# laboshinl/loam_velodyne

Measured on AMD Instinct MI355X. Metric: sweeps/sec (64-ring, 1M-pt map): feature extraction + odometry + scan-to-map registration, higher is better.
Workload: dtype f32

## Files before the change

loam_velodyne_amd/csrc/registration.hip:

```cpp
#include "registration.hpp"
#include "pinned_copy.hpp"
#include <atomic>
#include <chrono>
#include "scan.hpp"
#include "voxel.hpp"

namespace loamx {

__global__ __launch_bounds__(256) void k_stack(const float4* __restrict__ in, const float4* const* __restrict__ src, uint32_t n,
                                               const uint32_t* __restrict__ seg_off, uint32_t nseg, const Pose* __restrict__ poses,
                                               float inv_corner, float inv_surf, float4* __restrict__ stack, int* __restrict__ ijk,
                                               int* __restrict__ seg_minmax) {
  const uint32_t i = blockIdx.x * blockDim.x + threadIdx.x;
  const bool active = i < n;
  uint32_t seg = 0;
  int ix = 0, iy = 0, iz = 0;
  if (active) {
    seg = vox_find_seg(seg_off, nseg, i);
    const Pose T = poses[seg >> 1];
    const float4 p = src ? src[seg][i - seg_off[seg]] : in[i];
    float x = p.x, y = p.y, z = p.z;
    to_map(T, x, y, z);
    to_be_mapped(T, x, y, z);
    stack[i] = make_float4(x, y, z, p.w);
// ... 757 lines not shown

static double host_us() {
  return std::chrono::duration<double, std::micro>(std::chrono::steady_clock::now().time_since_epoch()).count();
}
struct Registrar::RunTrace {
  bool on;
  double t0, front = 0, first_gn = 0, callback = 0;
  int looks = 0;
};
#ifdef LOAMX_PROF_GN
static DevBuf<unsigned long long> g_gn_dbg;
#endif

void Registrar::enqueue_full(int mode) {
  if (!n_full_) return;
  if (mode == 1 && ++full_tag_ == 0u) full_tag_ = 1u;
  const uint32_t* skip = run_.vb_unchecked ? vb_.d_fail_word() : nullptr;
  hipLaunchKernelGGL(k_transform_full, dim3((n_full_ + 255) / 256), dim3(256), 0, st_, full_.p, n_full_, d_full_off_, n_sweeps_, poses_.p,
                     stats_.p, full_done_.p, mode, full_tag_, skip, vb_.epoch());
}

void Registrar::enqueue_front(bool legacy) {
  const uint32_t ns = n_sweeps_, nseg = 2 * ns, n = n_in_;
  hipLaunchKernelGGL(k_pose_init, dim3((ns + 63) / 64), dim3(64), 0, st_, d_guess_, ns, poses_.p, stats_.p, vox_.seg_minmax(), arrive_.p,
                     full_done_.p);
  if (n == 0) {
    LX_HIP(hipMemsetAsync(ds_off_.p, 0, sizeof(uint32_t) * (nseg + 1), st_));
    return;
  }
  if (legacy) {
    const uint32_t nb = (n + 255) / 256;
    hipLaunchKernelGGL(k_stack, dim3(nb), dim3(256), 0, st_, in_.p, d_src_, n, d_seg_off_, nseg, poses_.p, 1.0f / params.corner_leaf,
                       1.0f / params.surf_leaf, stack_.p, vox_.ijk(), vox_.seg_minmax());
    vox_.sort_reduce(stack_.p, nullptr, n, d_seg_off_, nseg, ds_pts_.p, ds_off_.p);
  } else {
    vb_.run(in_.p, d_src_, n, d_seg_off_, h_seg_off_.data(), nseg, poses_.p, 1.0f / params.corner_leaf, 1.0f / params.surf_leaf, stack_.p,
            ds_pts_.p, ds_off_.p);
  }
}

bool Registrar::wait_for_mirrors() {
  const bool no_poll = diag_env("LOAMX_NO_MIRROR_POLL") != nullptr;
  if (no_poll) { LX_HIP(hipEventSynchronize(ev_look_)); return false; }
  const uint32_t ns = n_sweeps_;
  const volatile SweepStats* hs = h_stats_.p;
  for (unsigned spin = 0;; spin++) {
    bool all = true;
    for (uint32_t k = 0; k < ns && all; k++) all = hs[k].done != 0;
    if (all) {
      std::atomic_thread_fence(std::memory_order_acquire);
      for (uint32_t k = 0; k < ns && all; k++) {
        SweepStats st;
        Pose T;
        memcpy(&st, (const void*)&h_stats_.p[k], sizeof(st));
        memcpy(&T, (const void*)&h_poses_.p[k], sizeof(T));
        all = st.pad1 == mirror_check_word(st, T);
      }
      if (all) return true;
    }
    if ((spin & 15) == 15) {
// ... 385 lines not shown
```

loam_velodyne_amd/csrc/voxbucket.hip:

```cpp
#include "voxbucket.hpp"
#include "scan.hpp"
#include "voxel.hpp"

namespace loamx {

struct VbArgs {
  const float4* in;
  const float4* const* src;
  const uint32_t* seg_off;
  const Pose* poses;
  VbSeg* segs;
  unsigned long long* lo;
  uint32_t* bseg;
  int* box;
  uint32_t* cnt;
  uint32_t* heads;
  uint32_t* ctl;
  uint32_t* h_fail;
  uint32_t* elems;
  float4* stack;
  float4* out;
  uint32_t* out_off;
  uint32_t n, nseg, nb, epoch;
  float inv_even, inv_odd;
  unsigned long long* dbg;
};

__device__ inline uint32_t vb_bits(unsigned long long v) { return v ? 64u - (uint32_t)__builtin_clzll(v) : 0u; }
__device__ inline void vb_fail(const VbArgs& A, int reason) {
  A.ctl[0] = A.epoch;
  A.h_fail[0] = A.epoch;
  A.h_fail[2 + reason] = A.epoch;
}
__device__ inline void vb_fail_reduce(const VbArgs& A, int reason) {
  vb_fail(A, reason);
  __hip_atomic_store(&A.ctl[0], A.epoch, __ATOMIC_RELAXED, __HIP_MEMORY_SCOPE_AGENT);
}
__device__ inline uint32_t vb_arrive(const VbArgs& A) {
  xchg_stores_done();
  return __hip_atomic_fetch_add(&A.ctl[1], 1u, __ATOMIC_RELAXED, __HIP_MEMORY_SCOPE_AGENT);
}
__device__ inline void vb_arrive_last(const VbArgs& A, uint32_t before) {
  if (before + 1u != A.nb) return;
  __hip_atomic_store(&A.ctl[1], 0u, __ATOMIC_RELAXED, __HIP_MEMORY_SCOPE_AGENT);
  if (__hip_atomic_load(&A.ctl[0], __ATOMIC_RELAXED, __HIP_MEMORY_SCOPE_AGENT) != A.epoch) return;
  for (uint32_t s = 0; s <= A.nseg; s++) __hip_atomic_store(&A.out_off[s], 0u, __ATOMIC_RELAXED, __HIP_MEMORY_SCOPE_AGENT);
}
constexpr int VB_OFF = 1 << 20;
__device__ inline bool vb_voxel(float v, float inv, int& i) {
  const float f = floorf(v * inv);
  if (!(fabsf(f) < (float)VB_OFF)) return false;
  i = (int)f;
  return true;
}
__device__ inline unsigned long long vb_key(int ix, int iy, int iz) {
  return ((unsigned long long)(uint32_t)(iz + VB_OFF) << 42) | ((unsigned long long)(uint32_t)(iy + VB_OFF) << 21) | (unsigned long long)(uint32_t)(ix + VB_OFF);
}

__global__ __launch_bounds__(VB_SAMPLE) void k_vb_plan(const VbArgs A) {
  __shared__ unsigned long long s_key[VB_SAMPLE], s_sorted[VB_SAMPLE];
  __shared__ uint32_t s_scan[17];
  __shared__ uint32_t s_bad;
  const int tid = (int)threadIdx.x;
  const uint32_t seg = blockIdx.x;
  const uint32_t a0 = A.seg_off[seg], ns = A.seg_off[seg + 1] - a0;
  const float4* __restrict__ pts = A.src ? A.src[seg] : A.in + a0;
  const float inv = (seg & 1) ? A.inv_odd : A.inv_even;
  uint32_t bucket0;
  {
    uint32_t part = 0;
    for (uint32_t s = (uint32_t)tid; s < seg; s += VB_SAMPLE) {
      const uint32_t m = A.seg_off[s + 1] - A.seg_off[s];
      part += m ? (m + VB_T - 1) / VB_T : 1u;
    }
    uint32_t tot;
    (void)block_excl_scan(part, s_scan, tot);
    bucket0 = tot;
  }
  const uint32_t nbuckets = ns ? (ns + VB_T - 1) / VB_T : 1u;
  const uint32_t m = ns < (uint32_t)VB_SAMPLE ? ns : (uint32_t)VB_SAMPLE;
  if (tid == 0) s_bad = nbuckets > (uint32_t)VB_SAMPLE ? 2u : 0u;
  __syncthreads();
  unsigned long long key = ~0ull;
  if (nbuckets > 1u && (uint32_t)tid < m) {
    const float4 p = pts[(uint32_t)(((unsigned long long)tid * ns) / m)];
    int v[3];
    if (vb_voxel(p.x, inv, v[0]) && vb_voxel(p.y, inv, v[1]) && vb_voxel(p.z, inv, v[2])) key = vb_key(v[0], v[1], v[2]);
    else atomicOr(&s_bad, 1u);
  }
  s_key[tid] = key;
  __syncthreads();
  if (nbuckets > 1u && (uint32_t)tid < m) {
    uint32_t r = 0;
    for (uint32_t u = 0; u < m; u++) {
      const unsigned long long k = s_key[u];
      r += (k < key || (k == key && u < (uint32_t)tid)) ? 1u : 0u;
    }
    s_sorted[r] = key;
  }
  __syncthreads();
  const uint32_t bad = s_bad;
  if (bad && tid == 0) vb_fail(A, (bad & 2u) ? 1 : 0);
  for (uint32_t k = (uint32_t)tid; k < nbuckets && k < (uint32_t)VB_SAMPLE; k += VB_SAMPLE) {
    A.lo[bucket0 + k] = (k == 0u || bad) ? 0ull : s_sorted[(uint32_t)(((unsigned long long)k * m) / nbuckets)];
    A.bseg[bucket0 + k] = seg;
    A.cnt[bucket0 + k] = 0u;
    A.heads[bucket0 + k] = 0u;
  }
  if (tid < 6) A.box[6 * seg + tid] = tid < 3 ? 2147483647 : (-2147483647 - 1);
  if (tid == 0) {
    VbSeg P;
    P.bucket0 = bucket0;
    P.nbuckets = bad ? 0u : nbuckets;
    P.pos_bits = vb_bits(ns ? (unsigned long long)(ns - 1) : 0ull);
    if (P.pos_bits == 0) P.pos_bits = 1;
    P.pad = 0u;
    A.segs[seg] = P;
  }
}

__global__ __launch_bounds__(256) void k_vb_stack(const VbArgs A) {
  __shared__ unsigned long long s_lo[64];
  __shared__ uint32_t s_tag[256], s_cnt[256], s_gbase[256];
  const uint32_t i = blockIdx.x * blockDim.x + threadIdx.x;
  const int lane = (int)(threadIdx.x & 63);
  const uint32_t lead = vox_find_seg(A.seg_off, A.nseg, blockIdx.x * blockDim.x);
  const VbSeg PL = A.segs[lead];
  if (threadIdx.x < 64) s_lo[threadIdx.x] = threadIdx.x < PL.nbuckets ? A.lo[PL.bucket0 + threadIdx.x] : ~0ull;
  s_tag[threadIdx.x] = 0xffffffffu;
  s_cnt[threadIdx.x] = 0u;
  __syncthreads();
  bool act = i < A.n;
  uint32_t g = 0u, pos = 0u;
  if (act) {
    const uint32_t seg = vox_find_seg(A.seg_off, A.nseg, i);
    const uint32_t a0 = A.seg_off[seg];
    const Pose T = A.poses[seg >> 1];
    const float4 p = A.src ? A.src[seg][i - a0] : A.in[i];
    float x = p.x, y = p.y, z = p.z;
    to_map(T, x, y, z);
    to_be_mapped(T, x, y, z);
    A.stack[i] = make_float4(x, y, z, p.w);
    const float inv = (seg & 1) ? A.inv_odd : A.inv_even;
    int v[3];
    const VbSeg P = seg == lead ? PL : A.segs[seg];
    if (!(vb_voxel(x, inv, v[0]) && vb_voxel(y, inv, v[1]) && vb_voxel(z, inv, v[2])) || P.nbuckets == 0u) {
      vb_fail(A, 0);
      act = false;
    } else {
      const unsigned long long key = vb_key(v[0], v[1], v[2]);
      uint32_t lo = 0u, hi = P.nbuckets;
      if (seg == lead && P.nbuckets <= 64u) {
        while (hi - lo > 1u) { const uint32_t mid = (lo + hi) >> 1; if (s_lo[mid] <= key) lo = mid; else hi = mid; }
      } else {
        const unsigned long long* __restrict__ sp = A.lo + P.bucket0;
        while (hi - lo > 1u) { const uint32_t mid = (lo + hi) >> 1; if (sp[mid] <= key) lo = mid; else hi = mid; }
      }
      g = P.bucket0 + lo;
      pos = i - a0;
    }
  }
  unsigned long long rem = __ballot(act);
  uint32_t slot = 0u;
  bool direct = false;
  while (rem) {
    const int l0 = __builtin_ctzll(rem);
    const uint32_t g0 = (uint32_t)__shfl((int)g, l0, 64);
    const unsigned long long m = __ballot(act && g == g0);
    uint32_t base = 0u, dir = 0u;
    if (lane == l0) {
      const uint32_t h = g0 & 255u;
      const uint32_t old = atomicCAS(&s_tag[h], 0xffffffffu, g0);
      if (old == 0xffffffffu || old == g0) base = atomicAdd(&s_cnt[h], (uint32_t)__popcll(m));
      else { base = atomicAdd(&A.cnt[g0], (uint32_t)__popcll(m)); dir = 1u; }
    }
    base = (uint32_t)__shfl((int)base, l0, 64);
    dir = (uint32_t)__shfl((int)dir, l0, 64);
    if (act && g == g0) { slot = base + (uint32_t)__popcll(m & ((1ull << lane) - 1ull)); direct = dir != 0u; }
    rem &= ~m;
  }
  __syncthreads();
  if (s_tag[threadIdx.x] != 0xffffffffu) s_gbase[threadIdx.x] = atomicAdd(&A.cnt[s_tag[threadIdx.x]], s_cnt[threadIdx.x]);
  __syncthreads();
  if (act) {
    if (!direct) slot += s_gbase[g & 255u];
    if (slot < (uint32_t)VB_CAP) A.elems[(size_t)g * VB_CAP + slot] = pos;
    else vb_fail(A, 5);
  }
}

constexpr uint32_t VB_SPIN_LIMIT = 1u << 20;
#ifdef LOAMX_PROF_VB
#define VB_TS(k) do { if (threadIdx.x == 0) A.dbg[(size_t)blockIdx.x * 16 + (k)] = wall_clock64(); } while (0)
#else
#define VB_TS(k) do { } while (0)
#endif
constexpr int VB_THREADS = VB_CAP / 8, VB_WAVES = VB_THREADS / 64;

__global__ __launch_bounds__(VB_THREADS) void k_vb_reduce(const VbArgs A) {
  __shared__ float4 s_buf[VB_CAP + 1];
  unsigned long long* s_w = (unsigned long long*)s_buf;
  __shared__ uint32_t s_hbits[VB_CAP / 32 + 1];
  __shared__ uint32_t s_wcnt[VB_WAVES][256];
  __shared__ uint32_t s_base[256];
  __shared__ uint32_t s_scan[17];
  __shared__ int s_box[6];
  const int tid = (int)threadIdx.x, lane = tid & 63, wid = tid >> 6;
  const uint32_t b = blockIdx.x;
  VB_TS(0);
  if (__hip_atomic_load(&A.ctl[0], __ATOMIC_RELAXED, __HIP_MEMORY_SCOPE_AGENT) == A.epoch) {
    if (tid == 0) {
      __hip_atomic_store(&A.heads[b], 1u, __ATOMIC_RELAXED, __HIP_MEMORY_SCOPE_AGENT);
      vb_arrive_last(A, vb_arrive(A));
    }
    return;
  }
  const uint32_t seg = A.bseg[b];
  const uint32_t c = min(A.cnt[b], (uint32_t)VB_CAP);
  const VbSeg P = A.segs[seg];
  const uint32_t sbeg = A.seg_off[seg];
  const float inv = (seg & 1) ? A.inv_odd : A.inv_even;
  const uint32_t* __restrict__ e = A.elems + (size_t)b * VB_CAP;
  const uint32_t pbits = P.pos_bits;
  const unsigned long long pmask = (1ull << pbits) - 1ull;
  if (tid < 6) s_box[tid] = tid < 3 ? 2147483647 : (-2147483647 - 1);
  __syncthreads();
  uint32_t pos8[8];
  int vx[8], vy[8], vz[8];
  {
    float4 pt[8];
#pragma unroll
    for (int j = 0; j < 8; j++) {
      const uint32_t i = (uint32_t)(wid * 512 + j * 64 + lane);
      pos8[j] = i < c ? e[i] : 0u;
    }
#pragma unroll
    for (int j = 0; j < 8; j++) {
      const uint32_t i = (uint32_t)(wid * 512 + j * 64 + lane);
      pt[j] = i < c ? A.stack[sbeg + pos8[j]] : make_float4(0.f, 0.f, 0.f, 0.f);
    }
    int mn[3] = {2147483647, 2147483647, 2147483647}, mx[3] = {-2147483647 - 1, -2147483647 - 1, -2147483647 - 1};
#pragma unroll
    for (int j = 0; j < 8; j++) {
      const uint32_t i = (uint32_t)(wid * 512 + j * 64 + lane);
      vx[j] = vy[j] = vz[j] = 0;
      if (i < c) {
        (void)vb_voxel(pt[j].x, inv, vx[j]); (void)vb_voxel(pt[j].y, inv, vy[j]); (void)vb_voxel(pt[j].z, inv, vz[j]);
        mn[0] = vx[j] < mn[0] ? vx[j] : mn[0]; mx[0] = vx[j] > mx[0] ? vx[j] : mx[0];
        mn[1] = vy[j] < mn[1] ? vy[j] : mn[1]; mx[1] = vy[j] > mx[1] ? vy[j] : mx[1];
        mn[2] = vz[j] < mn[2] ? vz[j] : mn[2]; mx[2] = vz[j] > mx[2] ? vz[j] : mx[2];
      }
    }
#pragma unroll
    for (int a = 0; a < 3; a++) {
#pragma unroll
      for (int d = 32; d > 0; d >>= 1) {
        const int lo = __shfl_xor(mn[a], d, 64), hi = __shfl_xor(mx[a], d, 64);
        mn[a] = lo < mn[a] ? lo : mn[a];
        mx[a] = hi > mx[a] ? hi : mx[a];
      }
    }
    if (lane == 0 && (uint32_t)(wid * 512) < c) {
#pragma unroll
      for (int a = 0; a < 3; a++) { atomicMin(&s_box[a], mn[a]); atomicMax(&s_box[3 + a], mx[a]); }
    }
  }
  __syncthreads();
  VB_TS(1);
  unsigned long long dimx = 1ull, dimy = 1ull, dimz = 1ull;
  int bx0 = 0, by0 = 0, bz0 = 0;
  if (c) {
    bx0 = s_box[0]; by0 = s_box[1]; bz0 = s_box[2];
    dimx = (unsigned long long)(s_box[3] - bx0 + 1); dimy = (unsigned long long)(s_box[4] - by0 + 1); dimz = (unsigned long long)(s_box[5] - bz0 + 1);
    if (tid < 6) {
      if (tid < 3) atomicMin(&A.box[6 * seg + tid], s_box[tid]); else atomicMax(&A.box[6 * seg + tid], s_box[tid]);
    }
  }
  const uint32_t key_bits = vb_bits(dimx * dimy * dimz - 1ull);
  const uint32_t total_bits = (key_bits ? key_bits : 1u) + pbits;
  if (total_bits > 63u) {
    if (tid == 0) vb_fail_reduce(A, 3);
  }
  const uint32_t npass = total_bits > 63u ? 0u : (total_bits + 7u) / 8u;
  unsigned long long w[8];
#pragma unroll
  for (int j = 0; j < 8; j++) {
    const uint32_t i = (uint32_t)(wid * 512 + j * 64 + lane);
    const unsigned long long lin = (unsigned long long)(vx[j] - bx0) + dimx * ((unsigned long long)(vy[j] - by0) + dimy * (unsigned long long)(vz[j] - bz0));
    w[j] = i < c ? ((lin << pbits) | (unsigned long long)pos8[j]) : ~0ull;
  }
  const bool wave_has = (uint32_t)(wid * 512) < c;
  if (npass == 0u) {
#pragma unroll
    for (int j = 0; j < 8; j++) {
      const uint32_t i = (uint32_t)(wid * 512 + j * 64 + lane);
      if (i < c) s_w[i] = w[j];
    }
    __syncthreads();
  }
  for (uint32_t p = 0; p < npass; p++) {
    const uint32_t shift = 8u * p;
    VB_TS(2 + (p < 7u ? p : 7u));
    if (tid < 256) {
#pragma unroll
      for (int k = 0; k < VB_WAVES; k++) s_wcnt[k][tid] = 0u;
    }
    __syncthreads();
    uint32_t rank[8];
#pragma unroll
    for (int j = 0; j < 8; j++) rank[j] = 0u;
    if (wave_has) {
#pragma unroll
      for (int j = 0; j < 8; j++) {
        const uint32_t i = (uint32_t)(wid * 512 + j * 64 + lane);
        const bool in = i < c;
        const uint32_t d = (uint32_t)((w[j] >> shift) & 255ull);
        unsigned long long m = __ballot(in);
#pragma unroll
        for (int bit = 0; bit < 8; bit++) {
          const unsigned long long bal = __ballot((d >> bit) & 1u);
          m &= ((d >> bit) & 1u) ? bal : ~bal;
        }
        const unsigned long long below = m & ((1ull << lane) - 1ull);
        const int leader = __builtin_ctzll(m | (1ull << 63));
        uint32_t old = 0u;
        if (in && lane == leader) {
          old = s_wcnt[wid][d];
          s_wcnt[wid][d] = old + (uint32_t)__popcll(m);
        }
        old = (uint32_t)__shfl((int)old, leader, 64);
        rank[j] = old + (uint32_t)__popcll(below);
        __builtin_amdgcn_wave_barrier();
      }
    }
    __syncthreads();
    {
      uint32_t run = 0u;
      if (tid < 256) {
#pragma unroll
        for (int k = 0; k < VB_WAVES; k++) { const uint32_t v = s_wcnt[k][tid]; s_wcnt[k][tid] = run; run += v; }
      }
      uint32_t tot;
      const uint32_t ex = block_excl_scan(run, s_scan, tot);
      if (tid < 256) s_base[tid] = ex;
    }
    __syncthreads();
    if (wave_has) {
#pragma unroll
      for (int j = 0; j < 8; j++) {
        const uint32_t i = (uint32_t)(wid * 512 + j * 64 + lane);
        if (i < c) {
          const uint32_t d = (uint32_t)((w[j] >> shift) & 255ull);
          s_w[s_base[d] + s_wcnt[wid][d] + rank[j]] = w[j];
        }
      }
    }
    __syncthreads();
    if (p + 1 < npass) {
#pragma unroll
      for (int j = 0; j < 8; j++) {
        const uint32_t i = (uint32_t)(wid * 512 + j * 64 + lane);
        w[j] = i < c ? s_w[i] : ~0ull;
      }
    }
  }
  VB_TS(10);
  if (tid == 0) s_w[c] = ~0ull;
  __syncthreads();
  const uint32_t l0 = (uint32_t)tid * 8u;
  unsigned long long vox[8];
  float4 pt[8];
#pragma unroll
  for (int j = 0; j < 8; j++) {
    const uint32_t l = l0 + (uint32_t)j;
    const unsigned long long x = l < c ? s_w[l] : ~0ull;
    vox[j] = x >> pbits;
    pt[j] = l < c ? A.stack[sbeg + (uint32_t)(x & pmask)] : make_float4(0.f, 0.f, 0.f, 0.f);
  }
  bool head[8];
  uint32_t nh = 0u, hb = 0u;
  unsigned long long prev = (l0 == 0u || l0 > c) ? ~0ull : (s_w[l0 - 1u] >> pbits);
#pragma unroll
  for (int j = 0; j < 8; j++) {
    const uint32_t l = l0 + (uint32_t)j;
    head[j] = l < c && (l == 0u || vox[j] != prev);
    nh += head[j] ? 1u : 0u;
    hb |= (head[j] || l >= c) ? (1u << j) : 0u;
    prev = vox[j];
  }
  __syncthreads();
#pragma unroll
  for (int j = 0; j < 8; j++) s_buf[l0 + (uint32_t)j] = pt[j];
  ((unsigned char*)s_hbits)[tid] = (unsigned char)hb;
  if (tid == 0) ((unsigned char*)s_hbits)[VB_THREADS] = 0xffu;
  __syncthreads();
  VB_TS(11);
  uint32_t tot;
  const uint32_t ex = block_excl_scan(nh, s_scan, tot);
  if (tid == 0) {
    xchg_stores_done();
    __hip_atomic_store(&A.heads[b], tot + 1u, __ATOMIC_RELAXED, __HIP_MEMORY_SCOPE_AGENT);
  }
  uint32_t part = 0u;
  for (uint32_t t = (uint32_t)tid; t < b; t += VB_THREADS) {
    uint32_t v = __hip_atomic_load(&A.heads[t], __ATOMIC_RELAXED, __HIP_MEMORY_SCOPE_AGENT), spins = 0u;
    while (v == 0u) {
      __builtin_amdgcn_s_sleep(2);
      v = __hip_atomic_load(&A.heads[t], __ATOMIC_RELAXED, __HIP_MEMORY_SCOPE_AGENT);
      if (++spins > VB_SPIN_LIMIT) { A.h_fail[1] = 1u; v = 1u; }
    }
    part += v - 1u;
  }
  VB_TS(12);
  uint32_t base;
  (void)block_excl_scan(part, s_scan, base);
  if (tid == 0) {
    if (P.bucket0 == b) __hip_atomic_store(&A.out_off[seg], base, __ATOMIC_RELAXED, __HIP_MEMORY_SCOPE_AGENT);
    if (b + 1u == A.nb) __hip_atomic_store(&A.out_off[A.nseg], base + tot, __ATOMIC_RELAXED, __HIP_MEMORY_SCOPE_AGENT);
  }
  if (b + 1u == A.nb) {
    int through = 0;
    for (uint32_t s = (uint32_t)tid; s < A.nseg; s += VB_THREADS) {
      int bb[6];
#pragma unroll
      for (int k = 0; k < 6; k++) bb[k] = __hip_atomic_load(&A.box[6 * s + k], __ATOMIC_RELAXED, __HIP_MEMORY_SCOPE_AGENT);
      if (bb[3] >= bb[0]) {
        const long long dx = (long long)bb[3] - bb[0] + 1, dy = (long long)bb[4] - bb[1] + 1, dz = (long long)bb[5] - bb[2] + 1;
        if (dx * dy > 2147483647LL || dx * dy * dz > 2147483647LL) through = 1;
      }
    }
    if (__syncthreads_or(through) && tid == 0) vb_fail_reduce(A, 2);
  }
  const uint32_t arrived = tid == 0 ? vb_arrive(A) : 0u;
  uint32_t pos = base + ex;
#pragma unroll
  for (int j = 0; j < 8; j++) {
    if (head[j]) {
      float sx = 0.f + pt[j].x, sy = 0.f + pt[j].y, sz = 0.f + pt[j].z, si = 0.f + pt[j].w;
      uint32_t cntp = 1u;
      bool open = true;
#pragma unroll
      for (int q = j + 1; q < 8; q++) {
        open = open && vox[q] == vox[j];
        if (open) { sx += pt[q].x; sy += pt[q].y; sz += pt[q].z; si += pt[q].w; cntp++; }
      }
      if (open) {
        uint32_t l = l0 + 8u;
        while (open) {
          const uint32_t hbyte = ((const unsigned char*)s_hbits)[l >> 3];
          float4 ts[8];
#pragma unroll
          for (int q = 0; q < 8; q++) ts[q] = s_buf[min(l + (uint32_t)q, (uint32_t)VB_CAP)];
#pragma unroll
          for (int q = 0; q < 8; q++) {
            open = open && !((hbyte >> q) & 1u);
            if (open) { sx += ts[q].x; sy += ts[q].y; sz += ts[q].z; si += ts[q].w; cntp++; }
          }
          l += 8u;
        }
      }
#ifdef LOAMX_PROF_VB
      atomicMax((unsigned long long*)&A.dbg[(size_t)blockIdx.x * 16 + 14], (unsigned long long)cntp);
#endif
      const float cf = (float)cntp;
      A.out[pos] = make_float4(sx / cf, sy / cf, sz / cf, si / cf);
      pos++;
    }
  }
  if (tid == 0) vb_arrive_last(A, arrived);
  VB_TS(13);
}

void VoxBucket::run(const float4* in, const float4* const* d_src, uint32_t n, const uint32_t* d_seg_off, const uint32_t* h_seg_off, uint32_t nseg,
                    const Pose* d_poses, float inv_even, float inv_odd, float4* stack, float4* out, uint32_t* d_out_off) {
  LX_REQUIRE(fits(n, nseg), "internal: VoxBucket::run outside its limits");
  uint32_t nb = 0;
  for (uint32_t s = 0; s < nseg; s++) {
    const uint32_t m = h_seg_off[s + 1] - h_seg_off[s];
    nb += m ? (m + VB_T - 1) / VB_T : 1u;
  }
  nb_ = nb;
  segs_.reserve(nseg);
  lo_.reserve(nb);
  bseg_.reserve(nb);
  box_.reserve((size_t)6 * nseg);
  cnt_.reserve(nb);
  heads_.reserve(nb);
  elems_.reserve((size_t)nb * VB_CAP);
  if (!ctl_ready_) {
    ctl_.reserve(4);
    h_fail_.reserve(16);
    for (int k = 0; k < 16; k++) h_fail_.p[k] = 0u;
    LX_HIP(hipMemsetAsync(ctl_.p, 0, sizeof(uint32_t) * 4, st_));
    ctl_ready_ = true;
  }
  if (++epoch_ == 0u) epoch_ = 1u;
  VbArgs a;
  a.in = in; a.src = d_src; a.seg_off = d_seg_off; a.poses = d_poses;
  a.segs = segs_.p; a.lo = lo_.p; a.bseg = bseg_.p; a.box = box_.p; a.cnt = cnt_.p; a.heads = heads_.p;
  a.ctl = ctl_.p; a.h_fail = h_fail_.p; a.elems = elems_.p; a.stack = stack; a.out = out; a.out_off = d_out_off;
  a.n = n; a.nseg = nseg; a.nb = nb; a.epoch = epoch_;
  a.inv_even = inv_even; a.inv_odd = inv_odd;
  a.dbg = nullptr;
#ifdef LOAMX_PROF_VB
  static DevBuf<unsigned long long> dbg;
  dbg.reserve((size_t)nb * 16 + 16);
  LX_HIP(hipMemsetAsync(dbg.p, 0, sizeof(unsigned long long) * ((size_t)nb * 16), st_));
  a.dbg = dbg.p;
#endif
  hipLaunchKernelGGL(k_vb_plan, dim3(nseg), dim3(VB_SAMPLE), 0, st_, a);
  hipLaunchKernelGGL(k_vb_stack, dim3((n + 255) / 256), dim3(256), 0, st_, a);
  hipLaunchKernelGGL(k_vb_reduce, dim3(nb), dim3(VB_THREADS), 0, st_, a);
  LX_HIP(hipGetLastError());
#ifdef LOAMX_PROF_VB
  {
    std::vector<unsigned long long> h((size_t)nb * 16);
    LX_HIP(hipStreamSynchronize(st_));
    LX_HIP(hipMemcpy(h.data(), dbg.p, sizeof(unsigned long long) * h.size(), hipMemcpyDeviceToHost));
    unsigned long long t0 = ~0ull, t1 = 0;
    for (uint32_t b = 0; b < nb; b++) { if (h[16 * b]) t0 = std::min(t0, h[16 * b]); t1 = std::max(t1, h[16 * b + 13]); }
    fprintf(stderr, "[k_vb_reduce %u buckets, %.1f us first start -> last end] bucket: start | box | passes ... | sorted | heads | look-back | end (us since first start)\n", nb, (t1 - t0) * 0.01);
    uint32_t slow = 0;
    for (uint32_t b = 0; b < nb; b++) if (h[16 * b + 13] > h[16 * slow + 13]) slow = b;
    for (uint32_t b : {0u, nb / 4, nb / 2, nb - 1, slow}) {
      fprintf(stderr, "  b%-4u", b);
      for (int k = 0; k < 14; k++) if (h[16 * b + k]) fprintf(stderr, " %d:%.1f", k, (h[16 * b + k] - t0) * 0.01);
      fprintf(stderr, " longest run %llu", h[16 * b + 14]);
      fprintf(stderr, "\n");
    }
  }
#endif
}

uint32_t VoxBucket::why() const {
  uint32_t m = 0;
  for (int r = 0; r < 8; r++)
    if (((volatile uint32_t*)h_fail_.p)[2 + r] == epoch_) m |= 1u << r;
  return m;
}

void VoxBucket::check() {
  if (h_fail_.p && ((volatile uint32_t*)h_fail_.p)[1]) {
    h_fail_.p[1] = 0u;
    throw Error(LOAMX_E_HIP, "voxel grid: a look-back wait inside k_vb_reduce timed out");
  }
}

}
```

loam_velodyne_amd/csrc/voxbucket.hpp:

```cpp
#pragma once
#include "common.h"
#include "dev_math.hpp"

namespace loamx {

#ifndef VB_CAP_LOG2
#define VB_CAP_LOG2 12
#endif
constexpr int VB_CAP = 1 << VB_CAP_LOG2;
constexpr int VB_T = VB_CAP / 2;
constexpr int VB_SAMPLE = 512;
constexpr int VB_MAXSEG = 4096;

struct VbSeg {
  uint32_t bucket0;
  uint32_t nbuckets;
  uint32_t pos_bits;
  uint32_t pad;
};

class VoxBucket {
 public:
  void init(hipStream_t st) { st_ = st; }
  void run(const float4* in, const float4* const* d_src, uint32_t n, const uint32_t* d_seg_off, const uint32_t* h_seg_off, uint32_t nseg,
           const Pose* d_poses, float inv_even, float inv_odd, float4* stack, float4* out, uint32_t* d_out_off);
  static bool fits(uint32_t n, uint32_t nseg) { return nseg >= 1 && nseg <= (uint32_t)VB_MAXSEG && n >= 1 && n < (1u << 24); }
  bool failed() const { return h_fail_.p && *(volatile uint32_t*)h_fail_.p == epoch_; }
  const uint32_t* d_fail_word() const { return ctl_.p; }
  uint32_t epoch() const { return epoch_; }
  uint32_t why() const;
  void check();
  uint32_t last_buckets() const { return nb_; }
  const VbSeg* d_segs() const { return segs_.p; }
  const unsigned long long* d_lo() const { return lo_.p; }
  const uint32_t* d_cnt() const { return cnt_.p; }

 private:
  hipStream_t st_ = nullptr;
  DevBuf<VbSeg> segs_;
  DevBuf<unsigned long long> lo_;
  DevBuf<uint32_t> bseg_;
  DevBuf<int> box_;
  DevBuf<uint32_t> cnt_, heads_, ctl_;
  DevBuf<uint32_t> elems_;
  PinBuf<uint32_t> h_fail_;
  uint32_t epoch_ = 0, nb_ = 0;
  bool ctl_ready_ = false;
};

}
```

Baseline: 16160.

## Replace per-bucket element lists with 16-bit bucket tags and gather-side collection

The stack kernel no longer scatters 32-bit point positions into per-bucket capacity-sized element lists. It writes a 16-bit bucket tag per point plus a per-chunk bucket range. Each reduce block then scans its segment's tags, skipping chunks whose range excludes it, to collect its own points in order. Other changes: the plan kernel splits sample ranking across four blocks per segment, pose initialisation is folded into the plan kernel, the radix sort skips position bits, and voxel runs are summed per head instead of per thread. This trades a large scattered write buffer for repeated tag scans in the reduce blocks, and adds more complex code paths.

Result: faster. 16620 (median of 6 runs) (+2.9%).

```diff
diff --git a/loam_velodyne_amd/csrc/registration.hip b/loam_velodyne_amd/csrc/registration.hip
--- a/loam_velodyne_amd/csrc/registration.hip
+++ b/loam_velodyne_amd/csrc/registration.hip
@@ -803,8 +803,9 @@
 
 void Registrar::enqueue_front(bool legacy) {
   const uint32_t ns = n_sweeps_, nseg = 2 * ns, n = n_in_;
-  hipLaunchKernelGGL(k_pose_init, dim3((ns + 63) / 64), dim3(64), 0, st_, d_guess_, ns, poses_.p, stats_.p, vox_.seg_minmax(), arrive_.p,
-                     full_done_.p);
+  if (legacy || n == 0)
+    hipLaunchKernelGGL(k_pose_init, dim3((ns + 63) / 64), dim3(64), 0, st_, d_guess_, ns, poses_.p, stats_.p, vox_.seg_minmax(), arrive_.p,
+                       full_done_.p);
   if (n == 0) {
     LX_HIP(hipMemsetAsync(ds_off_.p, 0, sizeof(uint32_t) * (nseg + 1), st_));
     return;
@@ -815,8 +816,12 @@
                        1.0f / params.surf_leaf, stack_.p, vox_.ijk(), vox_.seg_minmax());
     vox_.sort_reduce(stack_.p, nullptr, n, d_seg_off_, nseg, ds_pts_.p, ds_off_.p);
   } else {
+    static_assert(sizeof(SweepStats) == 8 * sizeof(int), "VbPoseInit::stats clears eight words per sweep");
+    VbPoseInit init;
+    init.guess = d_guess_; init.poses = poses_.p; init.stats = reinterpret_cast<int*>(stats_.p); init.seg_minmax = vox_.seg_minmax();
+    init.ticket = arrive_.p; init.full_done = full_done_.p; init.ns = ns;
     vb_.run(in_.p, d_src_, n, d_seg_off_, h_seg_off_.data(), nseg, poses_.p, 1.0f / params.corner_leaf, 1.0f / params.surf_leaf, stack_.p,
-            ds_pts_.p, ds_off_.p);
+            ds_pts_.p, ds_off_.p, &init);
   }
 }
 
diff --git a/loam_velodyne_amd/csrc/voxbucket.hip b/loam_velodyne_amd/csrc/voxbucket.hip
--- a/loam_velodyne_amd/csrc/voxbucket.hip
+++ b/loam_velodyne_amd/csrc/voxbucket.hip
@@ -11,13 +11,15 @@
   const Pose* poses;
   VbSeg* segs;
   unsigned long long* lo;
-  uint32_t* bseg;
+  VbBk* bk;
   int* box;
   uint32_t* cnt;
   uint32_t* heads;
   uint32_t* ctl;
   uint32_t* h_fail;
-  uint32_t* elems;
+  uint16_t* bword;
+  uint2* crange;
+  VbPoseInit init;
   float4* stack;
   float4* out;
   uint32_t* out_off;
@@ -57,24 +59,42 @@
   return ((unsigned long long)(uint32_t)(iz + VB_OFF) << 42) | ((unsigned long long)(uint32_t)(iy + VB_OFF) << 21) | (unsigned long long)(uint32_t)(ix + VB_OFF);
 }
 
+constexpr int VB_PLAN_PARTS = 4, VB_PLAN_KEYS = VB_SAMPLE / VB_PLAN_PARTS;
 __global__ __launch_bounds__(VB_SAMPLE) void k_vb_plan(const VbArgs A) {
-  __shared__ unsigned long long s_key[VB_SAMPLE], s_sorted[VB_SAMPLE];
+  __shared__ alignas(16) unsigned long long s_key[VB_SAMPLE];
+  __shared__ uint32_t s_part[VB_PLAN_PARTS][VB_PLAN_KEYS];
   __shared__ uint32_t s_scan[17];
   __shared__ uint32_t s_bad;
   const int tid = (int)threadIdx.x;
-  const uint32_t seg = blockIdx.x;
+  const uint32_t seg = blockIdx.x / VB_PLAN_PARTS, part = blockIdx.x % VB_PLAN_PARTS;
   const uint32_t a0 = A.seg_off[seg], ns = A.seg_off[seg + 1] - a0;
   const float4* __restrict__ pts = A.src ? A.src[seg] : A.in + a0;
   const float inv = (seg & 1) ? A.inv_odd : A.inv_even;
+  if (A.init.guess && part == VB_PLAN_PARTS - 1 && !(seg & 1u) && (seg >> 1) < A.init.ns) {
+    const uint32_t s = seg >> 1;
+    if (tid < 12) {
+      A.init.seg_minmax[12 * s + tid] = (tid % 6) < 3 ? 2147483647 : (-2147483647 - 1);
+      const float* __restrict__ g = A.init.guess + 6 * s;
+      float v;
+      if (tid < 6) v = g[tid];
+      else {
+        const float ang = g[(tid - 6) >> 1];
+        v = (float)((tid & 1) ? cos((double)ang) : sin((double)ang));
+      }
+      reinterpret_cast<float*>(A.init.poses + s)[tid] = v;
+    }
+    if (tid >= 64 && tid < 72) A.init.stats[8 * s + (tid - 64)] = 0;
+    if (tid == 72) { A.init.ticket[s] = 0u; A.init.full_done[s] = 0u; }
+  }
   uint32_t bucket0;
   {
-    uint32_t part = 0;
+    uint32_t sum = 0;
     for (uint32_t s = (uint32_t)tid; s < seg; s += VB_SAMPLE) {
       const uint32_t m = A.seg_off[s + 1] - A.seg_off[s];
-      part += m ? (m + VB_T - 1) / VB_T : 1u;
+      sum += m ? (m + VB_T - 1) / VB_T : 1u;
     }
     uint32_t tot;
-    (void)block_excl_scan(part, s_scan, tot);
+    (void)block_excl_scan(sum, s_scan, tot);
     bucket0 = tot;
   }
   const uint32_t nbuckets = ns ? (ns + VB_T - 1) / VB_T : 1u;
@@ -90,20 +110,44 @@
   }
   s_key[tid] = key;
   __syncthreads();
-  if (nbuckets > 1u && (uint32_t)tid < m) {
+  const uint32_t bad = s_bad;
+  const uint32_t own = part * VB_PLAN_KEYS + ((uint32_t)tid % VB_PLAN_KEYS), quarter = (uint32_t)tid / VB_PLAN_KEYS;
+  const bool ranked = nbuckets > 1u && !bad && own < m;
+  if (ranked) {
+    const unsigned long long mine = s_key[own];
+    const ulonglong2* __restrict__ k2 = reinterpret_cast<const ulonglong2*>(s_key);
     uint32_t r = 0;
-    for (uint32_t u = 0; u < m; u++) {
-      const unsigned long long k = s_key[u];
-      r += (k < key || (k == key && u < (uint32_t)tid)) ? 1u : 0u;
-    }
-    s_sorted[r] = key;
-  }
-  __syncthreads();
-  const uint32_t bad = s_bad;
+    for (uint32_t u = quarter * VB_PLAN_KEYS; u < (quarter + 1u) * VB_PLAN_KEYS; u += 16u) {
+      ulonglong2 k[8];
+#pragma unroll
+      for (int q = 0; q < 8; q++) k[q] = k2[(u >> 1) + (uint32_t)q];
+#pragma unroll
+      for (int q = 0; q < 8; q++) {
+        const uint32_t ua = u + 2u * (uint32_t)q;
+        r += (k[q].x < mine || (k[q].x == mine && ua < own)) ? 1u : 0u;
+        r += (k[q].y < mine || (k[q].y == mine && ua + 1u < own)) ? 1u : 0u;
+      }
+    }
+    s_part[quarter][(uint32_t)tid % VB_PLAN_KEYS] = r;
+  }
+  __syncthreads();
+  if (ranked && tid < VB_PLAN_KEYS) {
+    uint32_t r = 0;
+#pragma unroll
+    for (int q = 0; q < VB_PLAN_PARTS; q++) r += s_part[q][tid];
+    const uint32_t k = (uint32_t)(((unsigned long long)r * nbuckets + m - 1u) / m);
+    if (k >= 1u && k < nbuckets && (uint32_t)(((unsigned long long)k * m) / nbuckets) == r) A.lo[bucket0 + k] = s_key[own];
+  }
+  if (part != 0u) return;
   if (bad && tid == 0) vb_fail(A, (bad & 2u) ? 1 : 0);
   for (uint32_t k = (uint32_t)tid; k < nbuckets && k < (uint32_t)VB_SAMPLE; k += VB_SAMPLE) {
-    A.lo[bucket0 + k] = (k == 0u || bad) ? 0ull : s_sorted[(uint32_t)(((unsigned long long)k * m) / nbuckets)];
-    A.bseg[bucket0 + k] = seg;
+    if (k == 0u || bad) A.lo[bucket0 + k] = 0ull;
+    VbBk K;
+    K.seg = seg; K.sbeg = a0; K.send = a0 + ns; K.bucket0 = bucket0;
+    K.pos_bits = vb_bits(ns ? (unsigned long long)(ns - 1) : 0ull);
+    if (K.pos_bits == 0) K.pos_bits = 1;
+    K.pad[0] = K.pad[1] = K.pad[2] = 0u;
+    A.bk[bucket0 + k] = K;
     A.cnt[bucket0 + k] = 0u;
     A.heads[bucket0 + k] = 0u;
   }
@@ -119,9 +163,10 @@
   }
 }
 
-__global__ __launch_bounds__(256) void k_vb_stack(const VbArgs A) {
+__global__ __launch_bounds__(VB_CHUNK) void k_vb_stack(const VbArgs A) {
   __shared__ unsigned long long s_lo[64];
   __shared__ uint32_t s_tag[256], s_cnt[256], s_gbase[256];
+  __shared__ uint32_t s_gmin, s_gmax;
   const uint32_t i = blockIdx.x * blockDim.x + threadIdx.x;
   const int lane = (int)(threadIdx.x & 63);
   const uint32_t lead = vox_find_seg(A.seg_off, A.nseg, blockIdx.x * blockDim.x);
@@ -129,9 +174,10 @@
   if (threadIdx.x < 64) s_lo[threadIdx.x] = threadIdx.x < PL.nbuckets ? A.lo[PL.bucket0 + threadIdx.x] : ~0ull;
   s_tag[threadIdx.x] = 0xffffffffu;
   s_cnt[threadIdx.x] = 0u;
+  if (threadIdx.x == 0) { s_gmin = 0xffffffffu; s_gmax = 0u; }
   __syncthreads();
   bool act = i < A.n;
-  uint32_t g = 0u, pos = 0u;
+  uint32_t g = 0u, rel = 0u;
   if (act) {
     const uint32_t seg = vox_find_seg(A.seg_off, A.nseg, i);
     const uint32_t a0 = A.seg_off[seg];
@@ -157,8 +203,19 @@
         while (hi - lo > 1u) { const uint32_t mid = (lo + hi) >> 1; if (sp[mid] <= key) lo = mid; else hi = mid; }
       }
       g = P.bucket0 + lo;
-      pos = i - a0;
-    }
+      rel = lo;
+    }
+    A.bword[i] = act ? (uint16_t)rel : VB_REFUSED;
+  }
+  {
+    uint32_t gmn = act ? g : 0xffffffffu, gmx = act ? g : 0u;
+#pragma unroll
+    for (int d = 32; d > 0; d >>= 1) {
+      const uint32_t a = (uint32_t)__shfl_xor((int)gmn, d, 64), b = (uint32_t)__shfl_xor((int)gmx, d, 64);
+      gmn = a < gmn ? a : gmn;
+      gmx = b > gmx ? b : gmx;
+    }
+    if (lane == 0 && gmn != 0xffffffffu) { atomicMin(&s_gmin, gmn); atomicMax(&s_gmax, gmx); }
   }
   unsigned long long rem = __ballot(act);
   uint32_t slot = 0u;
@@ -184,9 +241,9 @@
   __syncthreads();
   if (act) {
     if (!direct) slot += s_gbase[g & 255u];
-    if (slot < (uint32_t)VB_CAP) A.elems[(size_t)g * VB_CAP + slot] = pos;
-    else vb_fail(A, 5);
-  }
+    if (slot >= (uint32_t)VB_CAP) vb_fail(A, 5);
+  }
+  if (threadIdx.x == 0) A.crange[blockIdx.x] = make_uint2(s_gmin, s_gmax);
 }
 
 constexpr uint32_t VB_SPIN_LIMIT = 1u << 20;
@@ -196,14 +253,37 @@
 #define VB_TS(k) do { } while (0)
 #endif
 constexpr int VB_THREADS = VB_CAP / 8, VB_WAVES = VB_THREADS / 64;
+__device__ inline uint32_t vb_match8(const uint4& v, uint32_t want) {
+  const uint32_t w4[4] = {v.x, v.y, v.z, v.w};
+  uint32_t m = 0u;
+#pragma unroll
+  for (int h = 0; h < 4; h++) {
+    m |= ((w4[h] & 0xffffu) == want ? 1u : 0u) << (2 * h);
+    m |= ((w4[h] >> 16) == want ? 1u : 0u) << (2 * h + 1);
+  }
+  return m;
+}
+
+template <int W>
+__device__ inline void vb_sum_run(const unsigned long long* s_w, const float4* s_pts, uint32_t l, uint32_t l_end, uint32_t c, uint32_t emask,
+                                  float& sx, float& sy, float& sz, float& si) {
+  float4 ts[W];
+#pragma unroll
+  for (int q = 0; q < W; q++) ts[q] = s_pts[(uint32_t)s_w[min(l + (uint32_t)q, c)] & emask];
+#pragma unroll
+  for (int q = 0; q < W; q++) {
+    if (l + (uint32_t)q < l_end) { sx += ts[q].x; sy += ts[q].y; sz += ts[q].z; si += ts[q].w; }
+  }
+}
 
 __global__ __launch_bounds__(VB_THREADS) void k_vb_reduce(const VbArgs A) {
-  __shared__ float4 s_buf[VB_CAP + 1];
-  unsigned long long* s_w = (unsigned long long*)s_buf;
-  __shared__ uint32_t s_hbits[VB_CAP / 32 + 1];
+  __shared__ float4 s_pts[VB_CAP];
+  __shared__ alignas(16) unsigned long long s_w[VB_CAP + 8];
+  uint32_t* s_pos = (uint32_t*)s_w;
   __shared__ uint32_t s_wcnt[VB_WAVES][256];
   __shared__ uint32_t s_base[256];
   __shared__ uint32_t s_scan[17];
+  __shared__ uint32_t s_pk[VB_WAVES][4];
   __shared__ int s_box[6];
   const int tid = (int)threadIdx.x, lane = tid & 63, wid = tid >> 6;
   const uint32_t b = blockIdx.x;
@@ -215,36 +295,99 @@
     }
     return;
   }
-  const uint32_t seg = A.bseg[b];
-  const uint32_t c = min(A.cnt[b], (uint32_t)VB_CAP);
-  const VbSeg P = A.segs[seg];
-  const uint32_t sbeg = A.seg_off[seg];
+  const VbBk K = A.bk[b];
+  const uint32_t seg = K.seg, sbeg = K.sbeg, send = K.send;
   const float inv = (seg & 1) ? A.inv_odd : A.inv_even;
-  const uint32_t* __restrict__ e = A.elems + (size_t)b * VB_CAP;
-  const uint32_t pbits = P.pos_bits;
-  const unsigned long long pmask = (1ull << pbits) - 1ull;
+  const uint32_t pbits = K.pos_bits;
   if (tid < 6) s_box[tid] = tid < 3 ? 2147483647 : (-2147483647 - 1);
-  __syncthreads();
-  uint32_t pos8[8];
+  const uint32_t want = b - K.bucket0;
+  const uint32_t o0 = sbeg / 8u, o1 = send > sbeg ? (send + 7u) / 8u : o0;
+  const uint32_t nround = (o1 - o0 + 8u * (uint32_t)VB_THREADS - 1u) / (8u * (uint32_t)VB_THREADS);
+  const bool skip = nround > 1u;
+  const uint4* __restrict__ bw = reinterpret_cast<const uint4*>(A.bword);
+  uint32_t found = 0u;
+  for (uint32_t r = 0; r < nround; r++) {
+    uint4 v[8];
+#pragma unroll
+    for (int k = 0; k < 8; k++) {
+      const uint32_t o = o0 + (r * 8u + (uint32_t)k) * (uint32_t)VB_THREADS + (uint32_t)tid;
+      bool ld = o < o1;
+      if (ld && skip) {
+        const uint2 cr = A.crange[o / (VB_CHUNK / 8u)];
+        ld = b >= cr.x && b <= cr.y;
+      }
+      v[k] = ld ? bw[o] : make_uint4(~0u, ~0u, ~0u, ~0u);
+    }
+    uint32_t mk[8], pk[4] = {0u, 0u, 0u, 0u};
+#pragma unroll
+    for (int k = 0; k < 8; k++) {
+      const uint32_t o = o0 + (r * 8u + (uint32_t)k) * (uint32_t)VB_THREADS + (uint32_t)tid;
+      uint32_t m = 0u;
+      if (o < o1) {
+        const uint32_t i0 = o * 8u;
+        const uint32_t lo = sbeg > i0 ? sbeg - i0 : 0u;
+        const uint32_t hi = send - i0 < 8u ? send - i0 : 8u;
+        m = vb_match8(v[k], want) & (0xffu << lo) & (0xffu >> (8u - hi));
+      }
+      mk[k] = m;
+      pk[k >> 1] |= (uint32_t)__popc(m) << (16 * (k & 1));
+    }
+    uint32_t inc[4];
+#pragma unroll
+    for (int q = 0; q < 4; q++) {
+      inc[q] = wave_incl_scan(pk[q], lane);
+      if (lane == 63) s_pk[wid][q] = inc[q];
+    }
+    __syncthreads();
+    uint32_t before[4] = {0u, 0u, 0u, 0u}, all[4] = {0u, 0u, 0u, 0u};
+#pragma unroll
+    for (int u = 0; u < VB_WAVES; u++) {
+#pragma unroll
+      for (int q = 0; q < 4; q++) {
+        const uint32_t t = s_pk[u][q];
+        all[q] += t;
+        before[q] += u < wid ? t : 0u;
+      }
+    }
+    uint32_t step_base = found;
+#pragma unroll
+    for (int k = 0; k < 8; k++) {
+      const int q = k >> 1, sh = 16 * (k & 1);
+      uint32_t off = step_base + ((before[q] >> sh) & 0xffffu) + ((inc[q] >> sh) & 0xffffu) - ((pk[q] >> sh) & 0xffffu);
+      const uint32_t rel = (o0 + (r * 8u + (uint32_t)k) * (uint32_t)VB_THREADS + (uint32_t)tid) * 8u - sbeg;
+      uint32_t m = mk[k];
+      while (m) {
+        const uint32_t bit = (uint32_t)__builtin_ctz(m);
+        m &= m - 1u;
+        if (off < (uint32_t)VB_CAP) s_pos[off] = rel + bit;
+        off++;
+      }
+      step_base += (all[q] >> sh) & 0xffffu;
+    }
+    found = step_base;
+    __syncthreads();
+  }
+  const uint32_t c = min(found, (uint32_t)VB_CAP);
+  VB_TS(15);
+  const uint32_t S = ((c + (uint32_t)VB_CAP / 8u - 1u) / ((uint32_t)VB_CAP / 8u)) * 64u;
+  const uint32_t w0 = (uint32_t)wid * S;
+#define VB_SLOT(j) (w0 + (uint32_t)(j) * 64u + (uint32_t)lane)
+#define VB_LIVE(j, i) ((uint32_t)(j) * 64u < S && (i) < c)
   int vx[8], vy[8], vz[8];
   {
     float4 pt[8];
 #pragma unroll
     for (int j = 0; j < 8; j++) {
-      const uint32_t i = (uint32_t)(wid * 512 + j * 64 + lane);
-      pos8[j] = i < c ? e[i] : 0u;
-    }
+      const uint32_t i = VB_SLOT(j);
+      pt[j] = VB_LIVE(j, i) ? A.stack[sbeg + s_pos[i]] : make_float4(0.f, 0.f, 0.f, 0.f);
+    }
+    int mn[3] = {2147483647, 2147483647, 2147483647}, mx[3] = {-2147483647 - 1, -2147483647 - 1, -2147483647 - 1};
 #pragma unroll
     for (int j = 0; j < 8; j++) {
-      const uint32_t i = (uint32_t)(wid * 512 + j * 64 + lane);
-      pt[j] = i < c ? A.stack[sbeg + pos8[j]] : make_float4(0.f, 0.f, 0.f, 0.f);
-    }
-    int mn[3] = {2147483647, 2147483647, 2147483647}, mx[3] = {-2147483647 - 1, -2147483647 - 1, -2147483647 - 1};
-#pragma unroll
-    for (int j = 0; j < 8; j++) {
-      const uint32_t i = (uint32_t)(wid * 512 + j * 64 + lane);
+      const uint32_t i = VB_SLOT(j);
       vx[j] = vy[j] = vz[j] = 0;
-      if (i < c) {
+      if (VB_LIVE(j, i)) {
+        s_pts[i] = pt[j];
         (void)vb_voxel(pt[j].x, inv, vx[j]); (void)vb_voxel(pt[j].y, inv, vy[j]); (void)vb_voxel(pt[j].z, inv, vz[j]);
         mn[0] = vx[j] < mn[0] ? vx[j] : mn[0]; mx[0] = vx[j] > mx[0] ? vx[j] : mx[0];
         mn[1] = vy[j] < mn[1] ? vy[j] : mn[1]; mx[1] = vy[j] > mx[1] ? vy[j] : mx[1];
@@ -260,7 +403,7 @@
         mx[a] = hi > mx[a] ? hi : mx[a];
       }
     }
-    if (lane == 0 && (uint32_t)(wid * 512) < c) {
+    if (lane == 0 && w0 < c) {
 #pragma unroll
       for (int a = 0; a < 3; a++) { atomicMin(&s_box[a], mn[a]); atomicMax(&s_box[3 + a], mx[a]); }
     }
@@ -281,25 +424,27 @@
   if (total_bits > 63u) {
     if (tid == 0) vb_fail_reduce(A, 3);
   }
-  const uint32_t npass = total_bits > 63u ? 0u : (total_bits + 7u) / 8u;
+  const uint32_t ebits = pbits < (uint32_t)VB_CAP_LOG2 ? pbits : (uint32_t)VB_CAP_LOG2;
+  const uint32_t emask = (1u << ebits) - 1u;
+  const uint32_t npass = total_bits > 63u ? 0u : ((key_bits ? key_bits : 1u) + 7u) / 8u;
   unsigned long long w[8];
 #pragma unroll
   for (int j = 0; j < 8; j++) {
-    const uint32_t i = (uint32_t)(wid * 512 + j * 64 + lane);
+    const uint32_t i = VB_SLOT(j);
     const unsigned long long lin = (unsigned long long)(vx[j] - bx0) + dimx * ((unsigned long long)(vy[j] - by0) + dimy * (unsigned long long)(vz[j] - bz0));
-    w[j] = i < c ? ((lin << pbits) | (unsigned long long)pos8[j]) : ~0ull;
-  }
-  const bool wave_has = (uint32_t)(wid * 512) < c;
+    w[j] = VB_LIVE(j, i) ? ((lin << ebits) | (unsigned long long)i) : ~0ull;
+  }
+  const bool wave_has = w0 < c;
   if (npass == 0u) {
 #pragma unroll
     for (int j = 0; j < 8; j++) {
-      const uint32_t i = (uint32_t)(wid * 512 + j * 64 + lane);
-      if (i < c) s_w[i] = w[j];
+      const uint32_t i = VB_SLOT(j);
+      if (VB_LIVE(j, i)) s_w[i] = w[j];
     }
     __syncthreads();
   }
   for (uint32_t p = 0; p < npass; p++) {
-    const uint32_t shift = 8u * p;
+    const uint32_t shift = ebits + 8u * p;
     VB_TS(2 + (p < 7u ? p : 7u));
     if (tid < 256) {
 #pragma unroll
@@ -312,25 +457,27 @@
     if (wave_has) {
 #pragma unroll
       for (int j = 0; j < 8; j++) {
-        const uint32_t i = (uint32_t)(wid * 512 + j * 64 + lane);
-        const bool in = i < c;
-        const uint32_t d = (uint32_t)((w[j] >> shift) & 255ull);
-        unsigned long long m = __ballot(in);
-#pragma unroll
-        for (int bit = 0; bit < 8; bit++) {
-          const unsigned long long bal = __ballot((d >> bit) & 1u);
-          m &= ((d >> bit) & 1u) ? bal : ~bal;
+        if ((uint32_t)j * 64u < S) {
+          const uint32_t i = VB_SLOT(j);
+          const bool in = i < c;
+          const uint32_t d = (uint32_t)((w[j] >> shift) & 255ull);
+          unsigned long long m = __ballot(in);
+#pragma unroll
+          for (int bit = 0; bit < 8; bit++) {
+            const unsigned long long bal = __ballot((d >> bit) & 1u);
+            m &= ((d >> bit) & 1u) ? bal : ~bal;
+          }
+          const unsigned long long below = m & ((1ull << lane) - 1ull);
+          const int leader = __builtin_ctzll(m | (1ull << 63));
+          uint32_t old = 0u;
+          if (in && lane == leader) {
+            old = s_wcnt[wid][d];
+            s_wcnt[wid][d] = old + (uint32_t)__popcll(m);
+          }
+          old = (uint32_t)__shfl((int)old, leader, 64);
+          rank[j] = old + (uint32_t)__popcll(below);
+          __builtin_amdgcn_wave_barrier();
         }
-        const unsigned long long below = m & ((1ull << lane) - 1ull);
-        const int leader = __builtin_ctzll(m | (1ull << 63));
-        uint32_t old = 0u;
-        if (in && lane == leader) {
-          old = s_wcnt[wid][d];
-          s_wcnt[wid][d] = old + (uint32_t)__popcll(m);
-        }
-        old = (uint32_t)__shfl((int)old, leader, 64);
-        rank[j] = old + (uint32_t)__popcll(below);
-        __builtin_amdgcn_wave_barrier();
       }
     }
     __syncthreads();
@@ -348,8 +495,8 @@
     if (wave_has) {
 #pragma unroll
       for (int j = 0; j < 8; j++) {
-        const uint32_t i = (uint32_t)(wid * 512 + j * 64 + lane);
-        if (i < c) {
+        const uint32_t i = VB_SLOT(j);
+        if (VB_LIVE(j, i)) {
           const uint32_t d = (uint32_t)((w[j] >> shift) & 255ull);
           s_w[s_base[d] + s_wcnt[wid][d] + rank[j]] = w[j];
         }
@@ -359,44 +506,44 @@
     if (p + 1 < npass) {
 #pragma unroll
       for (int j = 0; j < 8; j++) {
-        const uint32_t i = (uint32_t)(wid * 512 + j * 64 + lane);
-        w[j] = i < c ? s_w[i] : ~0ull;
-      }
-    }
-  }
+        const uint32_t i = VB_SLOT(j);
+        w[j] = VB_LIVE(j, i) ? s_w[i] : ~0ull;
+      }
+    }
+  }
+#undef VB_SLOT
+#undef VB_LIVE
   VB_TS(10);
   if (tid == 0) s_w[c] = ~0ull;
   __syncthreads();
   const uint32_t l0 = (uint32_t)tid * 8u;
   unsigned long long vox[8];
-  float4 pt[8];
 #pragma unroll
   for (int j = 0; j < 8; j++) {
     const uint32_t l = l0 + (uint32_t)j;
-    const unsigned long long x = l < c ? s_w[l] : ~0ull;
-    vox[j] = x >> pbits;
-    pt[j] = l < c ? A.stack[sbeg + (uint32_t)(x & pmask)] : make_float4(0.f, 0.f, 0.f, 0.f);
+    vox[j] = (l < c ? s_w[l] : ~0ull) >> ebits;
   }
   bool head[8];
-  uint32_t nh = 0u, hb = 0u;
-  unsigned long long prev = (l0 == 0u || l0 > c) ? ~0ull : (s_w[l0 - 1u] >> pbits);
+  uint32_t nh = 0u;
+  unsigned long long prev = (l0 == 0u || l0 > c) ? ~0ull : (s_w[l0 - 1u] >> ebits);
 #pragma unroll
   for (int j = 0; j < 8; j++) {
     const uint32_t l = l0 + (uint32_t)j;
     head[j] = l < c && (l == 0u || vox[j] != prev);
     nh += head[j] ? 1u : 0u;
-    hb |= (head[j] || l >= c) ? (1u << j) : 0u;
     prev = vox[j];
   }
-  __syncthreads();
-#pragma unroll
-  for (int j = 0; j < 8; j++) s_buf[l0 + (uint32_t)j] = pt[j];
-  ((unsigned char*)s_hbits)[tid] = (unsigned char)hb;
-  if (tid == 0) ((unsigned char*)s_hbits)[VB_THREADS] = 0xffu;
-  __syncthreads();
   VB_TS(11);
   uint32_t tot;
   const uint32_t ex = block_excl_scan(nh, s_scan, tot);
+  uint16_t* s_head = (uint16_t*)s_wcnt;
+  {
+    uint32_t k = ex;
+#pragma unroll
+    for (int j = 0; j < 8; j++) {
+      if (head[j]) s_head[k++] = (uint16_t)(l0 + (uint32_t)j);
+    }
+  }
   if (tid == 0) {
     xchg_stores_done();
     __hip_atomic_store(&A.heads[b], tot + 1u, __ATOMIC_RELAXED, __HIP_MEMORY_SCOPE_AGENT);
@@ -415,7 +562,7 @@
   uint32_t base;
   (void)block_excl_scan(part, s_scan, base);
   if (tid == 0) {
-    if (P.bucket0 == b) __hip_atomic_store(&A.out_off[seg], base, __ATOMIC_RELAXED, __HIP_MEMORY_SCOPE_AGENT);
+    if (K.bucket0 == b) __hip_atomic_store(&A.out_off[seg], base, __ATOMIC_RELAXED, __HIP_MEMORY_SCOPE_AGENT);
     if (b + 1u == A.nb) __hip_atomic_store(&A.out_off[A.nseg], base + tot, __ATOMIC_RELAXED, __HIP_MEMORY_SCOPE_AGENT);
   }
   if (b + 1u == A.nb) {
@@ -432,47 +579,30 @@
     if (__syncthreads_or(through) && tid == 0) vb_fail_reduce(A, 2);
   }
   const uint32_t arrived = tid == 0 ? vb_arrive(A) : 0u;
-  uint32_t pos = base + ex;
-#pragma unroll
-  for (int j = 0; j < 8; j++) {
-    if (head[j]) {
-      float sx = 0.f + pt[j].x, sy = 0.f + pt[j].y, sz = 0.f + pt[j].z, si = 0.f + pt[j].w;
-      uint32_t cntp = 1u;
-      bool open = true;
-#pragma unroll
-      for (int q = j + 1; q < 8; q++) {
-        open = open && vox[q] == vox[j];
-        if (open) { sx += pt[q].x; sy += pt[q].y; sz += pt[q].z; si += pt[q].w; cntp++; }
-      }
-      if (open) {
-        uint32_t l = l0 + 8u;
-        while (open) {
-          const uint32_t hbyte = ((const unsigned char*)s_hbits)[l >> 3];
-          float4 ts[8];
-#pragma unroll
-          for (int q = 0; q < 8; q++) ts[q] = s_buf[min(l + (uint32_t)q, (uint32_t)VB_CAP)];
-#pragma unroll
-          for (int q = 0; q < 8; q++) {
-            open = open && !((hbyte >> q) & 1u);
-            if (open) { sx += ts[q].x; sy += ts[q].y; sz += ts[q].z; si += ts[q].w; cntp++; }
-          }
-          l += 8u;
-        }
-      }
 #ifdef LOAMX_PROF_VB
-      atomicMax((unsigned long long*)&A.dbg[(size_t)blockIdx.x * 16 + 14], (unsigned long long)cntp);
+  uint32_t longest = 0u;
 #endif
-      const float cf = (float)cntp;
-      A.out[pos] = make_float4(sx / cf, sy / cf, sz / cf, si / cf);
-      pos++;
-    }
-  }
+  for (uint32_t h = (uint32_t)tid; h < tot; h += (uint32_t)VB_THREADS) {
+    const uint32_t l_beg = s_head[h], l_end = h + 1u < tot ? (uint32_t)s_head[h + 1u] : c;
+    float sx = 0.f, sy = 0.f, sz = 0.f, si = 0.f;
+    vb_sum_run<4>(s_w, s_pts, l_beg, l_end, c, emask, sx, sy, sz, si);
+    for (uint32_t l = l_beg + 4u; l < l_end; l += 16u) vb_sum_run<16>(s_w, s_pts, l, l_end, c, emask, sx, sy, sz, si);
+#ifdef LOAMX_PROF_VB
+    longest = max(longest, l_end - l_beg);
+#endif
+    const float cf = (float)(l_end - l_beg);
+    A.out[base + h] = make_float4(sx / cf, sy / cf, sz / cf, si / cf);
+  }
+#ifdef LOAMX_PROF_VB
+  if (longest) atomicMax((unsigned long long*)&A.dbg[(size_t)blockIdx.x * 16 + 14], (unsigned long long)longest);
+#endif
   if (tid == 0) vb_arrive_last(A, arrived);
   VB_TS(13);
 }
 
 void VoxBucket::run(const float4* in, const float4* const* d_src, uint32_t n, const uint32_t* d_seg_off, const uint32_t* h_seg_off, uint32_t nseg,
-                    const Pose* d_poses, float inv_even, float inv_odd, float4* stack, float4* out, uint32_t* d_out_off) {
+                    const Pose* d_poses, float inv_even, float inv_odd, float4* stack, float4* out, uint32_t* d_out_off,
+                    const VbPoseInit* init) {
   LX_REQUIRE(fits(n, nseg), "internal: VoxBucket::run outside its limits");
   uint32_t nb = 0;
   for (uint32_t s = 0; s < nseg; s++) {
@@ -482,11 +612,13 @@
   nb_ = nb;
   segs_.reserve(nseg);
   lo_.reserve(nb);
-  bseg_.reserve(nb);
+  bk_.reserve(nb);
   box_.reserve((size_t)6 * nseg);
   cnt_.reserve(nb);
   heads_.reserve(nb);
-  elems_.reserve((size_t)nb * VB_CAP);
+  const uint32_t nchunk = (n + VB_CHUNK - 1) / VB_CHUNK;
+  bword_.reserve((size_t)nchunk * VB_CHUNK);
+  crange_.reserve(nchunk);
   if (!ctl_ready_) {
     ctl_.reserve(4);
     h_fail_.reserve(16);
@@ -497,10 +629,11 @@
   if (++epoch_ == 0u) epoch_ = 1u;
   VbArgs a;
   a.in = in; a.src = d_src; a.seg_off = d_seg_off; a.poses = d_poses;
-  a.segs = segs_.p; a.lo = lo_.p; a.bseg = bseg_.p; a.box = box_.p; a.cnt = cnt_.p; a.heads = heads_.p;
-  a.ctl = ctl_.p; a.h_fail = h_fail_.p; a.elems = elems_.p; a.stack = stack; a.out = out; a.out_off = d_out_off;
+  a.segs = segs_.p; a.lo = lo_.p; a.bk = bk_.p; a.box = box_.p; a.cnt = cnt_.p; a.heads = heads_.p;
+  a.ctl = ctl_.p; a.h_fail = h_fail_.p; a.bword = bword_.p; a.crange = crange_.p; a.stack = stack; a.out = out; a.out_off = d_out_off;
   a.n = n; a.nseg = nseg; a.nb = nb; a.epoch = epoch_;
   a.inv_even = inv_even; a.inv_odd = inv_odd;
+  a.init = init ? *init : VbPoseInit();
   a.dbg = nullptr;
 #ifdef LOAMX_PROF_VB
   static DevBuf<unsigned long long> dbg;
@@ -508,8 +641,8 @@
   LX_HIP(hipMemsetAsync(dbg.p, 0, sizeof(unsigned long long) * ((size_t)nb * 16), st_));
   a.dbg = dbg.p;
 #endif
-  hipLaunchKernelGGL(k_vb_plan, dim3(nseg), dim3(VB_SAMPLE), 0, st_, a);
-  hipLaunchKernelGGL(k_vb_stack, dim3((n + 255) / 256), dim3(256), 0, st_, a);
+  hipLaunchKernelGGL(k_vb_plan, dim3(nseg * VB_PLAN_PARTS), dim3(VB_SAMPLE), 0, st_, a);
+  hipLaunchKernelGGL(k_vb_stack, dim3(nchunk), dim3(VB_CHUNK), 0, st_, a);
   hipLaunchKernelGGL(k_vb_reduce, dim3(nb), dim3(VB_THREADS), 0, st_, a);
   LX_HIP(hipGetLastError());
 #ifdef LOAMX_PROF_VB
@@ -525,6 +658,7 @@
     for (uint32_t b : {0u, nb / 4, nb / 2, nb - 1, slow}) {
       fprintf(stderr, "  b%-4u", b);
       for (int k = 0; k < 14; k++) if (h[16 * b + k]) fprintf(stderr, " %d:%.1f", k, (h[16 * b + k] - t0) * 0.01);
+      if (h[16 * b + 15]) fprintf(stderr, " collected:%.1f", (h[16 * b + 15] - t0) * 0.01);
       fprintf(stderr, " longest run %llu", h[16 * b + 14]);
       fprintf(stderr, "\n");
     }
diff --git a/loam_velodyne_amd/csrc/voxbucket.hpp b/loam_velodyne_amd/csrc/voxbucket.hpp
--- a/loam_velodyne_amd/csrc/voxbucket.hpp
+++ b/loam_velodyne_amd/csrc/voxbucket.hpp
@@ -11,6 +11,8 @@
 constexpr int VB_T = VB_CAP / 2;
 constexpr int VB_SAMPLE = 512;
 constexpr int VB_MAXSEG = 4096;
+constexpr int VB_CHUNK = 256;
+constexpr uint16_t VB_REFUSED = 0xffffu;
 
 struct VbSeg {
   uint32_t bucket0;
@@ -19,11 +21,28 @@
   uint32_t pad;
 };
 
+struct VbPoseInit {
+  const float* guess = nullptr;
+  Pose* poses = nullptr;
+  int* stats = nullptr;
+  int* seg_minmax = nullptr;
+  uint32_t* ticket = nullptr;
+  uint32_t* full_done = nullptr;
+  uint32_t ns = 0;
+};
+
+struct alignas(16) VbBk {
+  uint32_t seg, sbeg, send;
+  uint32_t bucket0, pos_bits;
+  uint32_t pad[3];
+};
+
 class VoxBucket {
  public:
   void init(hipStream_t st) { st_ = st; }
   void run(const float4* in, const float4* const* d_src, uint32_t n, const uint32_t* d_seg_off, const uint32_t* h_seg_off, uint32_t nseg,
-           const Pose* d_poses, float inv_even, float inv_odd, float4* stack, float4* out, uint32_t* d_out_off);
+           const Pose* d_poses, float inv_even, float inv_odd, float4* stack, float4* out, uint32_t* d_out_off,
+           const VbPoseInit* init = nullptr);
   static bool fits(uint32_t n, uint32_t nseg) { return nseg >= 1 && nseg <= (uint32_t)VB_MAXSEG && n >= 1 && n < (1u << 24); }
   bool failed() const { return h_fail_.p && *(volatile uint32_t*)h_fail_.p == epoch_; }
   const uint32_t* d_fail_word() const { return ctl_.p; }
@@ -39,10 +58,11 @@
   hipStream_t st_ = nullptr;
   DevBuf<VbSeg> segs_;
   DevBuf<unsigned long long> lo_;
-  DevBuf<uint32_t> bseg_;
+  DevBuf<VbBk> bk_;
   DevBuf<int> box_;
   DevBuf<uint32_t> cnt_, heads_, ctl_;
-  DevBuf<uint32_t> elems_;
+  DevBuf<uint16_t> bword_;
+  DevBuf<uint2> crange_;
   PinBuf<uint32_t> h_fail_;
   uint32_t epoch_ = 0, nb_ = 0;
   bool ctl_ready_ = false;
```
